# RaptorMai/online-continual-learning

Hardware: NVIDIA H100
Metric: replay-step images/sec (ASER+SCR, ResNet18, CIFAR100) (higher is better)
Workload: dtype f32

## Files before the change

### online-continual-learning_b200/csrc/umma.cuh

```cuda
#pragma once
#include <stdint.h>

namespace b200ocl {
namespace umma {

__device__ __forceinline__ uint32_t smem_u32(const void* p) {
  return static_cast<uint32_t>(__cvta_generic_to_shared(p));
}

__device__ __forceinline__ int sw128_offset_f32(int row, int chunk16) {
  return (row >> 3) * 256 + (row & 7) * 32 + ((chunk16 ^ (row & 7)) << 2);
}

__device__ __forceinline__ int frag_row(int t, int i) { return ((t >> 5) << 4) + ((t & 31) >> 2) + ((i & 2) << 2); }
__device__ __forceinline__ int frag_col(int t, int i) { return ((i >> 2) << 3) + ((t & 3) << 1) + (i & 1); }

__device__ __forceinline__ uint64_t make_smem_desc_sw128(uint32_t smem_addr) {
  uint64_t d = 0;
  d |= (uint64_t)((smem_addr >> 4) & 0x3FFF);
  d |= (uint64_t)1 << 16;
  d |= (uint64_t)((1024 >> 4) & 0x3FFF) << 32;
  d |= (uint64_t)1 << 62;
  return d;
}

__device__ __forceinline__ void fence() { asm volatile("wgmma.fence.sync.aligned;\n" ::: "memory"); }
__device__ __forceinline__ void commit() { asm volatile("wgmma.commit_group.sync.aligned;\n" ::: "memory"); }
template <int N>
__device__ __forceinline__ void wait() { asm volatile("wgmma.wait_group.sync.aligned %0;\n" ::"n"(N) : "memory"); }
template <int R>
__device__ __forceinline__ void fence_regs(float (&d)[R]) {
#pragma unroll
  for (int i = 0; i < R; ++i) asm volatile("" : "+f"(d[i])::"memory");
}
template <int N>
__device__ __forceinline__ void reg_dealloc() { asm volatile("setmaxnreg.dec.sync.aligned.u32 %0;\n" ::"n"(N)); }
template <int N>
__device__ __forceinline__ void reg_alloc() { asm volatile("setmaxnreg.inc.sync.aligned.u32 %0;\n" ::"n"(N)); }
__device__ __forceinline__ void fence_proxy_async_smem() { asm volatile("fence.proxy.async.shared::cta;\n" ::); }

__device__ __forceinline__ void mbar_init(uint64_t* bar, uint32_t count) {
  asm volatile("mbarrier.init.shared::cta.b64 [%0], %1;\n" ::"r"(smem_u32(bar)), "r"(count));
}
__device__ __forceinline__ void fence_mbar_init() { asm volatile("fence.mbarrier_init.release.cluster;\n" ::); }
__device__ __forceinline__ bool mbar_wait(uint64_t* bar, uint32_t parity, uint32_t max_spins = (1u << 24)) {
  const uint32_t addr = smem_u32(bar);
#pragma unroll 1
  for (uint32_t i = 0; i < max_spins; ++i) {
    uint32_t done;
    asm volatile(
        "{\n\t.reg .pred p;\n\t"
        "mbarrier.try_wait.parity.shared::cta.b64 p, [%1], %2;\n\t"
        "selp.u32 %0, 1, 0, p;\n\t}\n"
        : "=r"(done)
        : "r"(addr), "r"(parity)
        : "memory");
    if (done) return true;
  }
  return false;
}
__device__ __forceinline__ void mbar_arrive(uint64_t* bar) {
  asm volatile("mbarrier.arrive.shared::cta.b64 _, [%0];\n" ::"r"(smem_u32(bar)) : "memory");
}

__device__ __forceinline__ void mbar_expect_tx(uint64_t* bar, uint32_t bytes) {
  asm volatile("mbarrier.arrive.expect_tx.shared::cta.b64 _, [%0], %1;\n" ::"r"(smem_u32(bar)), "r"(bytes)
               : "memory");
}
__device__ __forceinline__ void bulk_g2s(void* smem_dst, const void* gmem_src, uint32_t bytes, uint64_t* bar) {
  asm volatile(
      "cp.async.bulk.shared::cluster.global.mbarrier::complete_tx::bytes [%0], [%1], %2, [%3];\n" ::"r"(
          smem_u32(smem_dst)),
      "l"(gmem_src), "r"(bytes), "r"(smem_u32(bar))
      : "memory");
}

__device__ __forceinline__ bool elect_one_sync() {
  uint32_t pred;
  asm volatile(
      "{\n\t.reg .pred P;\n\t"
      "elect.sync _|P, 0xffffffff;\n\t"
      "selp.u32 %0, 1, 0, P;\n\t}\n"
      : "=r"(pred));
  return pred != 0;
}

template <int N>
__device__ __forceinline__ void mma_tf32_ss(float (&d)[N / 2], uint64_t desc_a, uint64_t desc_b, uint32_t accumulate);
template <int N>
__device__ __forceinline__ void mma_tf32_rs(float (&d)[N / 2], const uint32_t (&a)[4], uint64_t desc_b, uint32_t accumulate);

template <>
__device__ __forceinline__ void mma_tf32_ss<16>(float (&d)[8], uint64_t desc_a, uint64_t desc_b, uint32_t accumulate) {
  asm volatile(
      "{\n\t.reg .pred p;\n\t"
      "setp.ne.b32 p, %10, 0;\n\t"
      "wgmma.mma_async.sync.aligned.m64n16k8.f32.tf32.tf32 {%0,%1,%2,%3,%4,%5,%6,%7}, %8, %9, p, 1, 1;\n\t}\n"
      : "+f"(d[0]), "+f"(d[1]), "+f"(d[2]), "+f"(d[3]), "+f"(d[4]), "+f"(d[5]), "+f"(d[6]), "+f"(d[7])
      : "l"(desc_a), "l"(desc_b), "r"(accumulate));
}

template <>
__device__ __forceinline__ void mma_tf32_ss<32>(float (&d)[16], uint64_t desc_a, uint64_t desc_b, uint32_t accumulate) {
  asm volatile(
      "{\n\t.reg .pred p;\n\t"
      "setp.ne.b32 p, %18, 0;\n\t"
      "wgmma.mma_async.sync.aligned.m64n32k8.f32.tf32.tf32 {%0,%1,%2,%3,%4,%5,%6,%7,%8,%9,%10,%11,%12,%13,%14,%15}, %16, %17, p, 1, 1;\n\t}\n"
      : "+f"(d[0]), "+f"(d[1]), "+f"(d[2]), "+f"(d[3]), "+f"(d[4]), "+f"(d[5]), "+f"(d[6]), "+f"(d[7]), "+f"(d[8]), "+f"(d[9]), "+f"(d[10]), "+f"(d[11]), "+f"(d[12]), "+f"(d[13]), "+f"(d[14]), "+f"(d[15])
      : "l"(desc_a), "l"(desc_b), "r"(accumulate));
}

template <>
__device__ __forceinline__ void mma_tf32_ss<48>(float (&d)[24], uint64_t desc_a, uint64_t desc_b, uint32_t accumulate) {
  asm volatile(
      "{\n\t.reg .pred p;\n\t"
      "setp.ne.b32 p, %26, 0;\n\t"
      "wgmma.mma_async.sync.aligned.m64n48k8.f32.tf32.tf32 {%0,%1,%2,%3,%4,%5,%6,%7,%8,%9,%10,%11,%12,%13,%14,%15,%16,%17,%18,%19,%20,%21,%22,%23}, %24, %25, p, 1, 1;\n\t}\n"
      : "+f"(d[0]), "+f"(d[1]), "+f"(d[2]), "+f"(d[3]), "+f"(d[4]), "+f"(d[5]), "+f"(d[6]), "+f"(d[7]), "+f"(d[8]), "+f"(d[9]), "+f"(d[10]), "+f"(d[11]), "+f"(d[12]), "+f"(d[13]), "+f"(d[14]), "+f"(d[15]), "+f"(d[16]), "+f"(d[17]), "+f"(d[18]), "+f"(d[19]), "+f"(d[20]), "+f"(d[21]), "+f"(d[22]), "+f"(d[23])
      : "l"(desc_a), "l"(desc_b), "r"(accumulate));
}

template <>
__device__ __forceinline__ void mma_tf32_ss<80>(float (&d)[40], uint64_t desc_a, uint64_t desc_b, uint32_t accumulate) {
  asm volatile(
      "{\n\t.reg .pred p;\n\t"
      "setp.ne.b32 p, %42, 0;\n\t"
      "wgmma.mma_async.sync.aligned.m64n80k8.f32.tf32.tf32 {%0,%1,%2,%3,%4,%5,%6,%7,%8,%9,%10,%11,%12,%13,%14,%15,%16,%17,%18,%19,%20,%21,%22,%23,%24,%25,%26,%27,%28,%29,%30,%31,%32,%33,%34,%35,%36,%37,%38,%39}, %40, %41, p, 1, 1;\n\t}\n"
      : "+f"(d[0]), "+f"(d[1]), "+f"(d[2]), "+f"(d[3]), "+f"(d[4]), "+f"(d[5]), "+f"(d[6]), "+f"(d[7]), "+f"(d[8]), "+f"(d[9]), "+f"(d[10]), "+f"(d[11]), "+f"(d[12]), "+f"(d[13]), "+f"(d[14]), "+f"(d[15]), "+f"(d[16]), "+f"(d[17]), "+f"(d[18]), "+f"(d[19]), "+f"(d[20]), "+f"(d[21]), "+f"(d[22]), "+f"(d[23]), "+f"(d[24]), "+f"(d[25]), "+f"(d[26]), "+f"(d[27]), "+f"(d[28]), "+f"(d[29]), "+f"(d[30]), "+f"(d[31]), "+f"(d[32]), "+f"(d[33]), "+f"(d[34]), "+f"(d[35]), "+f"(d[36]), "+f"(d[37]), "+f"(d[38]), "+f"(d[39])
      : "l"(desc_a), "l"(desc_b), "r"(accumulate));
}

template <>
__device__ __forceinline__ void mma_tf32_rs<32>(float (&d)[16], const uint32_t (&a)[4], uint64_t desc_b, uint32_t accumulate) {
  asm volatile(
      "{\n\t.reg .pred p;\n\t"
      "setp.ne.b32 p, %21, 0;\n\t"
      "wgmma.mma_async.sync.aligned.m64n32k8.f32.tf32.tf32 {%0,%1,%2,%3,%4,%5,%6,%7,%8,%9,%10,%11,%12,%13,%14,%15}, {%16,%17,%18,%19}, %20, p, 1, 1;\n\t}\n"
      : "+f"(d[0]), "+f"(d[1]), "+f"(d[2]), "+f"(d[3]), "+f"(d[4]), "+f"(d[5]), "+f"(d[6]), "+f"(d[7]), "+f"(d[8]), "+f"(d[9]), "+f"(d[10]), "+f"(d[11]), "+f"(d[12]), "+f"(d[13]), "+f"(d[14]), "+f"(d[15])
      : "r"(a[0]), "r"(a[1]), "r"(a[2]), "r"(a[3]), "l"(desc_b), "r"(accumulate));
}

__device__ __forceinline__ float round_tf32(float x) {
  uint32_t r;
  asm("cvt.rna.tf32.f32 %0, %1;\n" : "=r"(r) : "f"(x));
  return __uint_as_float(r);
}
__device__ __forceinline__ void split_tf32(float x, float& hi, float& lo) {
  hi = round_tf32(x);
  lo = x - hi;
}

}
}
```

### online-continual-learning_b200/csrc/wgrad_tc.cu

```cuda
#include "common.cuh"
#include "umma.cuh"
#include "wgrad_tc.cuh"

namespace b200ocl {
namespace {

constexpr int WT_THREADS = 32 * 14;
constexpr int WT_PS = 2;
constexpr int WT_XP = 40;
constexpr int WT_DZ_BYTES = 128 * 128;

struct WtGeom {
  int wp, pp, prow, xbytes;
};
__host__ __device__ inline WtGeom wt_geom(int H, int W) {
  WtGeom g;
  g.wp = W + 2;
  g.pp = (H + 2) * (W + 2);
  g.prow = 128 + 2 * g.wp + 2;
  g.xbytes = ((g.prow + 1) * WT_XP * 4 + 1023) / 1024 * 1024;
  return g;
}

__device__ __forceinline__ void load_a(const float* xs, int r, int c, uint32_t (&hi)[4], uint32_t (&lo)[4]) {
  const float v[4] = {xs[r * WT_XP + c], xs[r * WT_XP + c + 8], xs[(r + 4) * WT_XP + c], xs[(r + 4) * WT_XP + c + 8]};
#pragma unroll
  for (int i = 0; i < 4; ++i) {
    float h, l;
    umma::split_tf32(v[i], h, l);
    hi[i] = __float_as_uint(h);
    lo[i] = __float_as_uint(l);
  }
}

__global__ void __launch_bounds__(WT_THREADS, 1) wgrad_tc_kernel(WgradTcArgs a, int tiles_m) {
  extern __shared__ __align__(1024) unsigned char smem_raw[];
  __shared__ __align__(8) uint64_t full[WT_PS], empty[WT_PS];
  __shared__ int s_fail;

  const int tid = threadIdx.x, warp = tid >> 5, lane = tid & 31;
  const WtGeom G = wt_geom(a.H, a.W);
  const int stage_bytes = 2 * WT_DZ_BYTES + G.xbytes;
  const int sl = blockIdx.y, cb = blockIdx.z;
  const int chain0 = blockIdx.x * a.chains_per_cta;
  const int chain1 = min(a.chains, chain0 + a.chains_per_cta);
  const int k_total = 9 * a.Cin;

  if (tid == 0) {
    for (int i = 0; i < WT_PS; ++i) {
      umma::mbar_init(&full[i], 128 + 64);
      umma::mbar_init(&empty[i], 8);
    }
    umma::fence_mbar_init();
    s_fail = 0;
  }
  __syncthreads();

  if (warp >= 12) {
    const int lt = tid - 32 * 12;
    const int ch = lt & 7, r0 = lt >> 3;
    const bool ch_real = cb * 32 + ch * 4 < a.Cout;
    const int hp = a.H + 2;
    int pc = 0;
    for (int chain = chain0; chain < chain1; ++chain) {
      const int t1 = min(tiles_m, (chain + 1) * a.tpc);
      for (int tile = chain * a.tpc; tile < t1; ++tile, ++pc) {
        float4 v[16];
        int img, yp, xp;
        {
          const int sp = tile * 128 + r0;
          img = sp / G.pp;
          const int rem = sp - img * G.pp;
          yp = rem / G.wp;
          xp = rem - yp * G.wp;
        }
#pragma unroll
        for (int i = 0; i < 16; ++i) {
          v[i] = make_float4(0.f, 0.f, 0.f, 0.f);
          if (ch_real && img < a.N && yp < a.H && xp < a.W)
            v[i] = __ldg(reinterpret_cast<const float4*>(a.dz + ((size_t)(img * a.H + yp) * a.W + xp) * a.Cout + cb * 32) + ch);
          xp += 8;
          while (xp >= G.wp) {
            xp -= G.wp;
            if (++yp == hp) {
              yp = 0;
              ++img;
            }
          }
        }
        const int ps = pc % WT_PS;
        if (!umma::mbar_wait(&empty[ps], (uint32_t)(((pc / WT_PS) & 1) ^ 1))) s_fail = 1;
        float* zh = reinterpret_cast<float*>(smem_raw + (size_t)ps * stage_bytes);
        float* zl = zh + WT_DZ_BYTES / 4;
#pragma unroll
        for (int i = 0; i < 16; ++i) {
          const int pos = r0 + 8 * i;
          const float e[4] = {v[i].x, v[i].y, v[i].z, v[i].w};
#pragma unroll
          for (int j = 0; j < 4; ++j) {
            float h, l;
            umma::split_tf32(e[j], h, l);
            const int off = (pos >> 5) * 1024 + umma::sw128_offset_f32(ch * 4 + j, (pos & 31) >> 2) + (pos & 3);
            zh[off] = h;
            zl[off] = l;
          }
        }
        umma::fence_proxy_async_smem();
        umma::mbar_arrive(&full[ps]);
      }
    }
  } else if (warp >= 8) {
    const int lt = tid - 32 * 8;
    const int ch = lt & 7, r0 = lt >> 3;
    const int ch_valid = min(32, a.Cin - sl * 32);
    const bool ch_real = ch * 4 < ch_valid;
    const int nrow = G.prow;
    const int hp = a.H + 2;
    int pc = 0;
    for (int chain = chain0; chain < chain1; ++chain) {
      const int t1 = min(tiles_m, (chain + 1) * a.tpc);
      for (int tile = chain * a.tpc; tile < t1; ++tile, ++pc) {
        float4 v[WT_LD_MAX];
        int img, yp, xp;
        {
          const int sp = tile * 128 + r0;
          img = sp / G.pp;
          const int rem = sp - img * G.pp;
          yp = rem / G.wp;
          xp = rem - yp * G.wp;
        }
#pragma unroll
        for (int i = 0; i < WT_LD_MAX; ++i) {
          v[i] = make_float4(0.f, 0.f, 0.f, 0.f);
          const int ri = r0 + 16 * i;
          if (ch_real && ri < nrow) {
            const int y = yp - 1, x = xp - 1;
            if (img < a.N && (unsigned)y < (unsigned)a.H && (unsigned)x < (unsigned)a.W)
              v[i] = __ldg(reinterpret_cast<const float4*>(a.x + ((size_t)(img * a.H + y) * a.W + x) * a.Cin + sl * 32) + ch);
          }
          xp += 16;
          while (xp >= G.wp) {
            xp -= G.wp;
            if (++yp == hp) {
              yp = 0;
              ++img;
            }
          }
        }
        const int ps = pc % WT_PS;
        if (!umma::mbar_wait(&empty[ps], (uint32_t)(((pc / WT_PS) & 1) ^ 1))) s_fail = 1;
        float* xs = reinterpret_cast<float*>(smem_raw + (size_t)ps * stage_bytes + 2 * WT_DZ_BYTES);
#pragma unroll
        for (int i = 0; i < WT_LD_MAX; ++i) {
          const int ri = r0 + 16 * i;
          if (ri < nrow) *reinterpret_cast<float4*>(xs + ri * WT_XP + ch * 4) = v[i];
        }
        umma::mbar_arrive(&full[ps]);
      }
    }
  } else {
    const int h = warp >> 2, wt = tid & 127;
    const int m0 = 64 * h + 16 * (warp & 3) + (lane >> 2);
    const int kw = m0 >> 5, c = m0 & 31, q = lane & 3;
    const int n_valid = min(32, a.Cout - cb * 32);
    int pc = 0;
    for (int chain = chain0; chain < chain1; ++chain) {
      float acc[3][16];
      const int t0 = chain * a.tpc, t1 = min(tiles_m, (chain + 1) * a.tpc);
      for (int tile = t0; tile < t1; ++tile, ++pc) {
        const int ps = pc % WT_PS;
        if (!umma::mbar_wait(&full[ps], (uint32_t)((pc / WT_PS) & 1))) s_fail = 1;
        const unsigned char* st = smem_raw + (size_t)ps * stage_bytes;
        const float* xs = reinterpret_cast<const float*>(st + 2 * WT_DZ_BYTES);
        const uint64_t dZ0 = umma::make_smem_desc_sw128(umma::smem_u32(st));
        constexpr uint32_t Z_LO = (uint32_t)WT_DZ_BYTES >> 4;
#pragma unroll 1
        for (int ks = 0; ks < 16; ++ks) {
          const uint64_t dZh = dZ0 + (uint64_t)((ks >> 2) * 256 + (ks & 3) * 2), dZl = dZh + Z_LO;
          uint32_t ah[3][4], al[3][4];
#pragma unroll
          for (int kh = 0; kh < 3; ++kh) load_a(xs, ks * 8 + q + kh * G.wp + kw, c, ah[kh], al[kh]);
          const uint32_t accumulate = (tile == t0 && ks == 0) ? 0u : 1u;
          umma::fence();
#pragma unroll
          for (int kh = 0; kh < 3; ++kh) {
            umma::mma_tf32_rs<32>(acc[kh], ah[kh], dZh, accumulate);
            umma::mma_tf32_rs<32>(acc[kh], ah[kh], dZl, 1u);
            umma::mma_tf32_rs<32>(acc[kh], al[kh], dZh, 1u);
          }
          umma::commit();
          umma::wait<0>();
        }
#pragma unroll
        for (int kh = 0; kh < 3; ++kh) umma::fence_regs(acc[kh]);
        if (lane == 0) umma::mbar_arrive(&empty[ps]);
      }
#pragma unroll
      for (int i = 0; i < 16; i += 2) {
        const int m = 64 * h + umma::frag_row(wt, i), co = umma::frag_col(wt, i);
        const int kwi = m >> 5, ci = sl * 32 + (m & 31);
        if (kwi < 3 && ci < a.Cin && co < n_valid) {
#pragma unroll
          for (int kh = 0; kh < 3; ++kh) {
            float* dst = a.part + ((size_t)chain * k_total + (size_t)(kh * 3 + kwi) * a.Cin + ci) * a.Cout + cb * 32 + co;
            *reinterpret_cast<float2*>(dst) = make_float2(acc[kh][i], acc[kh][i + 1]);
          }
        }
      }
    }
  }
  __syncthreads();
  if (s_fail && tid == 0) a.part[0] = __int_as_float(0x7fc00000);
}

__global__ void wgrad_tc_reduce_kernel(const float* __restrict__ part, int chains, int Cin, int Cout, float* __restrict__ dw) {
  const int e = blockIdx.x * blockDim.x + threadIdx.x;
  const int total = 9 * Cin * Cout;
  if (e >= total) return;
  const int k = e / Cout, co = e - k * Cout;
  const int tap = k / Cin, ci = k - tap * Cin;
  double s = 0.0;
  for (int sp = 0; sp < chains; ++sp) s += (double)part[(size_t)sp * total + e];
  dw[((size_t)co * Cin + ci) * 9 + tap] = (float)s;
}

}

int launch_wgrad_tc(const WgradTcArgs& a, const WgradTcCfg& g, cudaStream_t stream) {
  const WtGeom G = wt_geom(a.H, a.W);
  const size_t smem = (size_t)WT_PS * (2 * WT_DZ_BYTES + (size_t)G.xbytes) + 1024;
  B200OCL_CUDA(raise_smem_limit<wgrad_tc_kernel>(smem));
  const double M = (double)a.N * a.H * a.W;
  B200OCL_PROF("wgrad_tc", 2.0 * M * 9.0 * a.Cin * a.Cout, stream);
  wgrad_tc_kernel<<<dim3(g.ctas_x, g.slices, g.cout_blocks), WT_THREADS, smem, stream>>>(a, g.tiles);
  B200OCL_LAUNCHED();
  return B200OCL_OK;
}

}

extern "C" size_t b200ocl_wgrad_tc_selftest_workspace_bytes(int N, int H, int W, int cin, int cout) {
  using namespace b200ocl;
  if (N < 1 || H < 1 || W < 1 || cin < 1 || cout < 1) return 0;
  const WgradTcCfg g = wgrad_tc_cfg(N, H, W, 3, 1, 1, cin, cout, sm_count());
  if (!g.eligible) return 0;
  return align_up((size_t)g.chains * 9 * cin * cout * sizeof(float), 256);
}

extern "C" int b200ocl_wgrad_tc_selftest(const float* x, const float* dz, float* dw_oihw, int N, int H, int W, int cin, int cout,
                                         void* workspace, size_t workspace_bytes, void* stream_) {
  using namespace b200ocl;
  cudaStream_t stream = static_cast<cudaStream_t>(stream_);
  B200OCL_CHECK_ARG(x && dz && dw_oihw && N >= 1, "null pointer / empty batch");
  const WgradTcCfg g = wgrad_tc_cfg(N, H, W, 3, 1, 1, cin, cout, sm_count());
  if (!g.eligible) {
    set_error("b200ocl_wgrad_tc_selftest: geometry not covered (3x3 stride 1, W <= 37, channels %% 4 == 0)");
    return B200OCL_EUNSUPPORTED;
  }
  int rc = check_workspace("b200ocl_wgrad_tc_selftest", workspace, workspace_bytes,
                           b200ocl_wgrad_tc_selftest_workspace_bytes(N, H, W, cin, cout));
  if (rc) return rc;
  WgradTcArgs a{};
  a.x = x; a.dz = dz; a.part = static_cast<float*>(workspace);
  a.N = N; a.H = H; a.W = W; a.Cin = cin; a.Cout = cout;
  a.tpc = g.tpc; a.chains = g.chains; a.chains_per_cta = g.chains_per_cta;
  if ((rc = launch_wgrad_tc(a, g, stream))) return rc;
  const int total = 9 * cin * cout;
  wgrad_tc_reduce_kernel<<<(total + 255) / 256, 256, 0, stream>>>(a.part, g.chains, cin, cout, dw_oihw);
  B200OCL_LAUNCHED();
  return B200OCL_OK;
}
```

### online-continual-learning_b200/csrc/wgrad_tc.cuh

```cuda
#pragma once
#include <cuda_runtime.h>

namespace b200ocl {

constexpr int WT_LD_MAX = 13;

struct WgradTcCfg {
  int eligible;
  int slices;
  int cout_blocks;
  int tiles;
  int tpc;
  int chains;
  int chains_per_cta;
  int ctas_x;
};

inline int wgrad_tc_tiles(int N, int H, int W) {
  const long pp = (long)(H + 2) * (W + 2);
  const long last = (long)(N - 1) * pp + (long)(H - 1) * (W + 2) + (W - 1);
  return (int)(last / 128) + 1;
}

inline WgradTcCfg wgrad_tc_cfg(int N, int H, int W, int ks, int stride, int pad, int cin, int cout, int sms) {
  WgradTcCfg g{};
  g.eligible = (ks == 3 && stride == 1 && pad == 1 && cin % 4 == 0 && cout % 4 == 0 && cin >= 4 && cout >= 4 &&
                128 + 2 * (W + 2) + 2 <= 16 * WT_LD_MAX && (long)N * (H + 2) * (W + 2) < 2000000000L) ? 1 : 0;
  if (!g.eligible) return g;
  g.slices = (cin + 31) / 32;
  g.cout_blocks = (cout + 31) / 32;
  g.tiles = wgrad_tc_tiles(N, H, W);
  g.tpc = 2;
  g.chains = (g.tiles + g.tpc - 1) / g.tpc;
  int want = sms / (g.slices * g.cout_blocks);
  if (want < 1) want = 1;
  if (want > g.chains) want = g.chains;
  g.chains_per_cta = (g.chains + want - 1) / want;
  g.ctas_x = (g.chains + g.chains_per_cta - 1) / g.chains_per_cta;
  return g;
}

struct WgradTcArgs {
  const float* x;
  const float* dz;
  float* part;
  int N, H, W, Cin, Cout;
  int tpc, chains, chains_per_cta;
};

int launch_wgrad_tc(const WgradTcArgs& a, const WgradTcCfg& g, cudaStream_t stream);

}
```

Measured before the change: 2186.

## Restructure wgrad tensor-core kernel with variable N tiles and two consumer groups

Reworks the 3x3 weight-gradient wgmma kernel. The input-channel slice drops from 32 to 20 so all three kw taps fit in one 64-row M tile, and the output-channel tile becomes a templated 8-40 multiple chosen to fit Cout with less padding. The two consumer warpgroups now process independent chains, each with its own staged buffers (up to four stages), instead of splitting M. A/B fragment loads are double-buffered against in-flight wgmma groups (wait<1>), and register allocation is rebalanced with setmaxnreg. This adds template instantiations and more complex stage indexing, and it changes the grid shape (more slices), which could shift load balance.

Result: faster. 2343 (median of 6 runs) (+7.1%).

```diff
diff --git a/online-continual-learning_b200/csrc/umma.cuh b/online-continual-learning_b200/csrc/umma.cuh
--- a/online-continual-learning_b200/csrc/umma.cuh
+++ b/online-continual-learning_b200/csrc/umma.cuh
@@ -140,6 +140,46 @@
       : "r"(a[0]), "r"(a[1]), "r"(a[2]), "r"(a[3]), "l"(desc_b), "r"(accumulate));
 }
 
+template <>
+__device__ __forceinline__ void mma_tf32_rs<8>(float (&d)[4], const uint32_t (&a)[4], uint64_t desc_b, uint32_t accumulate) {
+  asm volatile(
+      "{\n\t.reg .pred p;\n\t"
+      "setp.ne.b32 p, %9, 0;\n\t"
+      "wgmma.mma_async.sync.aligned.m64n8k8.f32.tf32.tf32 {%0,%1,%2,%3}, {%4,%5,%6,%7}, %8, p, 1, 1;\n\t}\n"
+      : "+f"(d[0]), "+f"(d[1]), "+f"(d[2]), "+f"(d[3])
+      : "r"(a[0]), "r"(a[1]), "r"(a[2]), "r"(a[3]), "l"(desc_b), "r"(accumulate));
+}
+
+template <>
+__device__ __forceinline__ void mma_tf32_rs<16>(float (&d)[8], const uint32_t (&a)[4], uint64_t desc_b, uint32_t accumulate) {
+  asm volatile(
+      "{\n\t.reg .pred p;\n\t"
+      "setp.ne.b32 p, %13, 0;\n\t"
+      "wgmma.mma_async.sync.aligned.m64n16k8.f32.tf32.tf32 {%0,%1,%2,%3,%4,%5,%6,%7}, {%8,%9,%10,%11}, %12, p, 1, 1;\n\t}\n"
+      : "+f"(d[0]), "+f"(d[1]), "+f"(d[2]), "+f"(d[3]), "+f"(d[4]), "+f"(d[5]), "+f"(d[6]), "+f"(d[7])
+      : "r"(a[0]), "r"(a[1]), "r"(a[2]), "r"(a[3]), "l"(desc_b), "r"(accumulate));
+}
+
+template <>
+__device__ __forceinline__ void mma_tf32_rs<24>(float (&d)[12], const uint32_t (&a)[4], uint64_t desc_b, uint32_t accumulate) {
+  asm volatile(
+      "{\n\t.reg .pred p;\n\t"
+      "setp.ne.b32 p, %17, 0;\n\t"
+      "wgmma.mma_async.sync.aligned.m64n24k8.f32.tf32.tf32 {%0,%1,%2,%3,%4,%5,%6,%7,%8,%9,%10,%11}, {%12,%13,%14,%15}, %16, p, 1, 1;\n\t}\n"
+      : "+f"(d[0]), "+f"(d[1]), "+f"(d[2]), "+f"(d[3]), "+f"(d[4]), "+f"(d[5]), "+f"(d[6]), "+f"(d[7]), "+f"(d[8]), "+f"(d[9]), "+f"(d[10]), "+f"(d[11])
+      : "r"(a[0]), "r"(a[1]), "r"(a[2]), "r"(a[3]), "l"(desc_b), "r"(accumulate));
+}
+
+template <>
+__device__ __forceinline__ void mma_tf32_rs<40>(float (&d)[20], const uint32_t (&a)[4], uint64_t desc_b, uint32_t accumulate) {
+  asm volatile(
+      "{\n\t.reg .pred p;\n\t"
+      "setp.ne.b32 p, %25, 0;\n\t"
+      "wgmma.mma_async.sync.aligned.m64n40k8.f32.tf32.tf32 {%0,%1,%2,%3,%4,%5,%6,%7,%8,%9,%10,%11,%12,%13,%14,%15,%16,%17,%18,%19}, {%20,%21,%22,%23}, %24, p, 1, 1;\n\t}\n"
+      : "+f"(d[0]), "+f"(d[1]), "+f"(d[2]), "+f"(d[3]), "+f"(d[4]), "+f"(d[5]), "+f"(d[6]), "+f"(d[7]), "+f"(d[8]), "+f"(d[9]), "+f"(d[10]), "+f"(d[11]), "+f"(d[12]), "+f"(d[13]), "+f"(d[14]), "+f"(d[15]), "+f"(d[16]), "+f"(d[17]), "+f"(d[18]), "+f"(d[19])
+      : "r"(a[0]), "r"(a[1]), "r"(a[2]), "r"(a[3]), "l"(desc_b), "r"(accumulate));
+}
+
 __device__ __forceinline__ float round_tf32(float x) {
   uint32_t r;
   asm("cvt.rna.tf32.f32 %0, %1;\n" : "=r"(r) : "f"(x));
diff --git a/online-continual-learning_b200/csrc/wgrad_tc.cu b/online-continual-learning_b200/csrc/wgrad_tc.cu
--- a/online-continual-learning_b200/csrc/wgrad_tc.cu
+++ b/online-continual-learning_b200/csrc/wgrad_tc.cu
@@ -5,10 +5,12 @@
 namespace b200ocl {
 namespace {
 
-constexpr int WT_THREADS = 32 * 14;
-constexpr int WT_PS = 2;
-constexpr int WT_XP = 40;
-constexpr int WT_DZ_BYTES = 128 * 128;
+constexpr int WT_THREADS = 32 * 16;
+constexpr int WT_PS_MAX = 4;
+constexpr int WT_XP = 24;
+constexpr size_t WT_SMEM_LIMIT = 227 * 1024 - 1024;
+
+__host__ __device__ constexpr int wt_dz_bytes(int bn) { return 4 * bn * 128; }
 
 struct WtGeom {
   int wp, pp, prow, xbytes;
@@ -18,191 +20,206 @@
   g.wp = W + 2;
   g.pp = (H + 2) * (W + 2);
   g.prow = 128 + 2 * g.wp + 2;
-  g.xbytes = ((g.prow + 1) * WT_XP * 4 + 1023) / 1024 * 1024;
+  g.xbytes = (g.prow * WT_XP * 4 + 1023) / 1024 * 1024;
   return g;
 }
 
-__device__ __forceinline__ void load_a(const float* xs, int r, int c, uint32_t (&hi)[4], uint32_t (&lo)[4]) {
-  const float v[4] = {xs[r * WT_XP + c], xs[r * WT_XP + c + 8], xs[(r + 4) * WT_XP + c], xs[(r + 4) * WT_XP + c + 8]};
-#pragma unroll
-  for (int i = 0; i < 4; ++i) {
-    float h, l;
-    umma::split_tf32(v[i], h, l);
-    hi[i] = __float_as_uint(h);
-    lo[i] = __float_as_uint(l);
-  }
-}
-
-__global__ void __launch_bounds__(WT_THREADS, 1) wgrad_tc_kernel(WgradTcArgs a, int tiles_m) {
+__host__ __device__ inline int wt_stage_bytes(const WtGeom& G, int bn) { return 2 * wt_dz_bytes(bn) + G.xbytes; }
+
+__device__ __forceinline__ void load_a(const float* xs, int p, int wp, int o0, int o1, uint32_t (&hi)[3][4],
+                                       uint32_t (&lo)[3][4]) {
+#pragma unroll
+  for (int kh = 0; kh < 3; ++kh) {
+    const float* r = xs + (p + kh * wp) * WT_XP;
+    const float v[4] = {r[o0], r[o1], r[4 * WT_XP + o0], r[4 * WT_XP + o1]};
+#pragma unroll
+    for (int i = 0; i < 4; ++i) {
+      float h, l;
+      umma::split_tf32(v[i], h, l);
+      hi[kh][i] = __float_as_uint(h);
+      lo[kh][i] = __float_as_uint(l);
+    }
+  }
+}
+
+template <int BN>
+__device__ __forceinline__ void issue_step(float (&acc)[3][BN / 2], const uint32_t (&hi)[3][4], const uint32_t (&lo)[3][4],
+                                           uint64_t dZh, uint64_t dZl, uint32_t accumulate) {
+  umma::fence();
+#pragma unroll
+  for (int kh = 0; kh < 3; ++kh) {
+    umma::mma_tf32_rs<BN>(acc[kh], hi[kh], dZh, accumulate);
+    umma::mma_tf32_rs<BN>(acc[kh], hi[kh], dZl, 1u);
+    umma::mma_tf32_rs<BN>(acc[kh], lo[kh], dZh, 1u);
+  }
+  umma::commit();
+}
+
+__device__ __forceinline__ int wt_row_kw(int m) { return min(m / WT_SLICE, 2); }
+
+template <int BN>
+__global__ void __launch_bounds__(WT_THREADS, 1) wgrad_tc_kernel(WgradTcArgs a, int tiles_m, int stages) {
   extern __shared__ __align__(1024) unsigned char smem_raw[];
-  __shared__ __align__(8) uint64_t full[WT_PS], empty[WT_PS];
+  __shared__ __align__(8) uint64_t full[WT_PS_MAX], empty[WT_PS_MAX];
   __shared__ int s_fail;
+  constexpr int DZ_BYTES = wt_dz_bytes(BN);
+  constexpr int SUB = BN * 128;
 
   const int tid = threadIdx.x, warp = tid >> 5, lane = tid & 31;
   const WtGeom G = wt_geom(a.H, a.W);
-  const int stage_bytes = 2 * WT_DZ_BYTES + G.xbytes;
+  const int stage_bytes = wt_stage_bytes(G, BN);
+  const int per = stages >> 1;
   const int sl = blockIdx.y, cb = blockIdx.z;
   const int chain0 = blockIdx.x * a.chains_per_cta;
   const int chain1 = min(a.chains, chain0 + a.chains_per_cta);
   const int k_total = 9 * a.Cin;
 
   if (tid == 0) {
-    for (int i = 0; i < WT_PS; ++i) {
-      umma::mbar_init(&full[i], 128 + 64);
-      umma::mbar_init(&empty[i], 8);
+    for (int i = 0; i < stages; ++i) {
+      umma::mbar_init(&full[i], 128 + 128);
+      umma::mbar_init(&empty[i], 4);
     }
     umma::fence_mbar_init();
     s_fail = 0;
   }
   __syncthreads();
 
-  if (warp >= 12) {
-    const int lt = tid - 32 * 12;
-    const int ch = lt & 7, r0 = lt >> 3;
-    const bool ch_real = cb * 32 + ch * 4 < a.Cout;
-    const int hp = a.H + 2;
-    int pc = 0;
-    for (int chain = chain0; chain < chain1; ++chain) {
-      const int t1 = min(tiles_m, (chain + 1) * a.tpc);
-      for (int tile = chain * a.tpc; tile < t1; ++tile, ++pc) {
-        float4 v[16];
-        int img, yp, xp;
-        {
-          const int sp = tile * 128 + r0;
-          img = sp / G.pp;
-          const int rem = sp - img * G.pp;
-          yp = rem / G.wp;
-          xp = rem - yp * G.wp;
+  if (warp >= 8) {
+    umma::reg_dealloc<96>();
+    const bool dz_loader = warp >= 12;
+    int pc0 = 0, pc1 = 0;
+    for (int c2 = chain0; c2 < chain1; c2 += 2) {
+      for (int tt = 0; tt < a.tpc; ++tt) {
+#pragma unroll 1
+        for (int h = 0; h < 2; ++h) {
+          const int chain = c2 + h, tile = chain * a.tpc + tt;
+          if (chain >= chain1 || tile >= tiles_m) continue;
+          const int n = h ? pc1++ : pc0++;
+          const int ps = h + 2 * (n % per);
+          const uint32_t parity = (uint32_t)(((n / per) & 1) ^ 1);
+          unsigned char* st = smem_raw + (size_t)ps * stage_bytes;
+          if (dz_loader) {
+            const int pos = tid - 32 * 12;
+            constexpr int NC = BN / 4;
+            float4 v[NC];
+            {
+              const int sp = tile * 128 + pos;
+              const int img = sp / G.pp, rem = sp - img * G.pp;
+              const int yp = rem / G.wp, xp = rem - yp * G.wp;
+              const bool pix = img < a.N && yp < a.H && xp < a.W;
+              const float* src = a.dz + ((size_t)(img * a.H + yp) * a.W + xp) * a.Cout + cb * BN;
+#pragma unroll
+              for (int j = 0; j < NC; ++j) {
+                v[j] = make_float4(0.f, 0.f, 0.f, 0.f);
+                if (pix && cb * BN + 4 * j < a.Cout) v[j] = __ldg(reinterpret_cast<const float4*>(src) + j);
+              }
+            }
+            if (!umma::mbar_wait(&empty[ps], parity)) s_fail = 1;
+            float* zh = reinterpret_cast<float*>(st);
+            float* zl = zh + DZ_BYTES / 4;
+#pragma unroll
+            for (int j = 0; j < NC; ++j) {
+              const float e[4] = {v[j].x, v[j].y, v[j].z, v[j].w};
+#pragma unroll
+              for (int k = 0; k < 4; ++k) {
+                float hv, lv;
+                umma::split_tf32(e[k], hv, lv);
+                const int off = (pos >> 5) * (SUB / 4) + umma::sw128_offset_f32(4 * j + k, (pos & 31) >> 2) + (pos & 3);
+                zh[off] = hv;
+                zl[off] = lv;
+              }
+            }
+            umma::fence_proxy_async_smem();
+          } else {
+            const int lt = tid - 32 * 8;
+            const int ch = lt & 7, r0 = lt >> 3;
+            const bool ch_real = ch * 4 < min(WT_SLICE, a.Cin - sl * WT_SLICE);
+            const int hp = a.H + 2;
+            float4 v[WT_LD_MAX];
+            int img, yp, xp;
+            {
+              const int sp = tile * 128 + r0;
+              img = sp / G.pp;
+              const int rem = sp - img * G.pp;
+              yp = rem / G.wp;
+              xp = rem - yp * G.wp;
+            }
+#pragma unroll
+            for (int i = 0; i < WT_LD_MAX; ++i) {
+              v[i] = make_float4(0.f, 0.f, 0.f, 0.f);
+              const int ri = r0 + 16 * i;
+              if (ch_real && ri < G.prow) {
+                const int y = yp - 1, x = xp - 1;
+                if (img < a.N && (unsigned)y < (unsigned)a.H && (unsigned)x < (unsigned)a.W)
+                  v[i] = __ldg(reinterpret_cast<const float4*>(a.x + ((size_t)(img * a.H + y) * a.W + x) * a.Cin +
+                                                               sl * WT_SLICE + ch * 4));
+              }
+              xp += 16;
+              while (xp >= G.wp) {
+                xp -= G.wp;
+                if (++yp == hp) {
+                  yp = 0;
+                  ++img;
+                }
+              }
+            }
+            if (!umma::mbar_wait(&empty[ps], parity)) s_fail = 1;
+            float* xs = reinterpret_cast<float*>(st + 2 * DZ_BYTES);
+            if (ch < WT_XP / 4) {
+#pragma unroll
+              for (int i = 0; i < WT_LD_MAX; ++i) {
+                const int ri = r0 + 16 * i;
+                if (ri < G.prow) *reinterpret_cast<float4*>(xs + ri * WT_XP + ch * 4) = v[i];
+              }
+            }
+          }
+          umma::mbar_arrive(&full[ps]);
         }
-#pragma unroll
-        for (int i = 0; i < 16; ++i) {
-          v[i] = make_float4(0.f, 0.f, 0.f, 0.f);
-          if (ch_real && img < a.N && yp < a.H && xp < a.W)
-            v[i] = __ldg(reinterpret_cast<const float4*>(a.dz + ((size_t)(img * a.H + yp) * a.W + xp) * a.Cout + cb * 32) + ch);
-          xp += 8;
-          while (xp >= G.wp) {
-            xp -= G.wp;
-            if (++yp == hp) {
-              yp = 0;
-              ++img;
-            }
-          }
-        }
-        const int ps = pc % WT_PS;
-        if (!umma::mbar_wait(&empty[ps], (uint32_t)(((pc / WT_PS) & 1) ^ 1))) s_fail = 1;
-        float* zh = reinterpret_cast<float*>(smem_raw + (size_t)ps * stage_bytes);
-        float* zl = zh + WT_DZ_BYTES / 4;
-#pragma unroll
-        for (int i = 0; i < 16; ++i) {
-          const int pos = r0 + 8 * i;
-          const float e[4] = {v[i].x, v[i].y, v[i].z, v[i].w};
-#pragma unroll
-          for (int j = 0; j < 4; ++j) {
-            float h, l;
-            umma::split_tf32(e[j], h, l);
-            const int off = (pos >> 5) * 1024 + umma::sw128_offset_f32(ch * 4 + j, (pos & 31) >> 2) + (pos & 3);
-            zh[off] = h;
-            zl[off] = l;
-          }
-        }
-        umma::fence_proxy_async_smem();
-        umma::mbar_arrive(&full[ps]);
-      }
-    }
-  } else if (warp >= 8) {
-    const int lt = tid - 32 * 8;
-    const int ch = lt & 7, r0 = lt >> 3;
-    const int ch_valid = min(32, a.Cin - sl * 32);
-    const bool ch_real = ch * 4 < ch_valid;
-    const int nrow = G.prow;
-    const int hp = a.H + 2;
-    int pc = 0;
-    for (int chain = chain0; chain < chain1; ++chain) {
-      const int t1 = min(tiles_m, (chain + 1) * a.tpc);
-      for (int tile = chain * a.tpc; tile < t1; ++tile, ++pc) {
-        float4 v[WT_LD_MAX];
-        int img, yp, xp;
-        {
-          const int sp = tile * 128 + r0;
-          img = sp / G.pp;
-          const int rem = sp - img * G.pp;
-          yp = rem / G.wp;
-          xp = rem - yp * G.wp;
-        }
-#pragma unroll
-        for (int i = 0; i < WT_LD_MAX; ++i) {
-          v[i] = make_float4(0.f, 0.f, 0.f, 0.f);
-          const int ri = r0 + 16 * i;
-          if (ch_real && ri < nrow) {
-            const int y = yp - 1, x = xp - 1;
-            if (img < a.N && (unsigned)y < (unsigned)a.H && (unsigned)x < (unsigned)a.W)
-              v[i] = __ldg(reinterpret_cast<const float4*>(a.x + ((size_t)(img * a.H + y) * a.W + x) * a.Cin + sl * 32) + ch);
-          }
-          xp += 16;
-          while (xp >= G.wp) {
-            xp -= G.wp;
-            if (++yp == hp) {
-              yp = 0;
-              ++img;
-            }
-          }
-        }
-        const int ps = pc % WT_PS;
-        if (!umma::mbar_wait(&empty[ps], (uint32_t)(((pc / WT_PS) & 1) ^ 1))) s_fail = 1;
-        float* xs = reinterpret_cast<float*>(smem_raw + (size_t)ps * stage_bytes + 2 * WT_DZ_BYTES);
-#pragma unroll
-        for (int i = 0; i < WT_LD_MAX; ++i) {
-          const int ri = r0 + 16 * i;
-          if (ri < nrow) *reinterpret_cast<float4*>(xs + ri * WT_XP + ch * 4) = v[i];
-        }
-        umma::mbar_arrive(&full[ps]);
       }
     }
   } else {
+    umma::reg_alloc<160>();
     const int h = warp >> 2, wt = tid & 127;
-    const int m0 = 64 * h + 16 * (warp & 3) + (lane >> 2);
-    const int kw = m0 >> 5, c = m0 & 31, q = lane & 3;
-    const int n_valid = min(32, a.Cout - cb * 32);
+    const int g = 16 * (warp & 3) + (lane >> 2), q = lane & 3;
+    const int kw0 = wt_row_kw(g), kw1 = wt_row_kw(g + 8);
+    const int o0 = kw0 * WT_XP + g - WT_SLICE * kw0, o1 = kw1 * WT_XP + g + 8 - WT_SLICE * kw1;
+    const int n_valid = min(BN, a.Cout - cb * BN);
+    constexpr uint32_t Z_LO = (uint32_t)DZ_BYTES >> 4;
     int pc = 0;
-    for (int chain = chain0; chain < chain1; ++chain) {
-      float acc[3][16];
+    for (int chain = chain0 + h; chain < chain1; chain += 2) {
+      float acc[3][BN / 2];
       const int t0 = chain * a.tpc, t1 = min(tiles_m, (chain + 1) * a.tpc);
       for (int tile = t0; tile < t1; ++tile, ++pc) {
-        const int ps = pc % WT_PS;
-        if (!umma::mbar_wait(&full[ps], (uint32_t)((pc / WT_PS) & 1))) s_fail = 1;
+        const int ps = h + 2 * (pc % per);
+        if (!umma::mbar_wait(&full[ps], (uint32_t)((pc / per) & 1))) s_fail = 1;
         const unsigned char* st = smem_raw + (size_t)ps * stage_bytes;
-        const float* xs = reinterpret_cast<const float*>(st + 2 * WT_DZ_BYTES);
+        const float* xs = reinterpret_cast<const float*>(st + 2 * DZ_BYTES);
         const uint64_t dZ0 = umma::make_smem_desc_sw128(umma::smem_u32(st));
-        constexpr uint32_t Z_LO = (uint32_t)WT_DZ_BYTES >> 4;
+        auto dz_desc = [&](int ks) { return dZ0 + (uint64_t)(((ks >> 2) * SUB + (ks & 3) * 32) >> 4); };
+        uint32_t ah[2][3][4], al[2][3][4];
+        load_a(xs, q, G.wp, o0, o1, ah[0], al[0]);
 #pragma unroll 1
-        for (int ks = 0; ks < 16; ++ks) {
-          const uint64_t dZh = dZ0 + (uint64_t)((ks >> 2) * 256 + (ks & 3) * 2), dZl = dZh + Z_LO;
-          uint32_t ah[3][4], al[3][4];
-#pragma unroll
-          for (int kh = 0; kh < 3; ++kh) load_a(xs, ks * 8 + q + kh * G.wp + kw, c, ah[kh], al[kh]);
-          const uint32_t accumulate = (tile == t0 && ks == 0) ? 0u : 1u;
-          umma::fence();
-#pragma unroll
-          for (int kh = 0; kh < 3; ++kh) {
-            umma::mma_tf32_rs<32>(acc[kh], ah[kh], dZh, accumulate);
-            umma::mma_tf32_rs<32>(acc[kh], ah[kh], dZl, 1u);
-            umma::mma_tf32_rs<32>(acc[kh], al[kh], dZh, 1u);
-          }
-          umma::commit();
-          umma::wait<0>();
+        for (int ks = 0; ks < 16; ks += 2) {
+          issue_step<BN>(acc, ah[0], al[0], dz_desc(ks), dz_desc(ks) + Z_LO, (tile == t0 && ks == 0) ? 0u : 1u);
+          umma::wait<1>();
+          load_a(xs, (ks + 1) * 8 + q, G.wp, o0, o1, ah[1], al[1]);
+          issue_step<BN>(acc, ah[1], al[1], dz_desc(ks + 1), dz_desc(ks + 1) + Z_LO, 1u);
+          umma::wait<1>();
+          load_a(xs, min(ks + 2, 15) * 8 + q, G.wp, o0, o1, ah[0], al[0]);
         }
+        umma::wait<0>();
 #pragma unroll
         for (int kh = 0; kh < 3; ++kh) umma::fence_regs(acc[kh]);
         if (lane == 0) umma::mbar_arrive(&empty[ps]);
       }
 #pragma unroll
-      for (int i = 0; i < 16; i += 2) {
-        const int m = 64 * h + umma::frag_row(wt, i), co = umma::frag_col(wt, i);
-        const int kwi = m >> 5, ci = sl * 32 + (m & 31);
-        if (kwi < 3 && ci < a.Cin && co < n_valid) {
+      for (int i = 0; i < BN / 2; i += 2) {
+        const int m = umma::frag_row(wt, i), co = umma::frag_col(wt, i);
+        const int kwi = wt_row_kw(m), c = m - WT_SLICE * kwi, ci = sl * WT_SLICE + c;
+        if (c < WT_SLICE && ci < a.Cin && co < n_valid) {
 #pragma unroll
           for (int kh = 0; kh < 3; ++kh) {
-            float* dst = a.part + ((size_t)chain * k_total + (size_t)(kh * 3 + kwi) * a.Cin + ci) * a.Cout + cb * 32 + co;
+            float* dst = a.part + ((size_t)chain * k_total + (size_t)(kh * 3 + kwi) * a.Cin + ci) * a.Cout + cb * BN + co;
             *reinterpret_cast<float2*>(dst) = make_float2(acc[kh][i], acc[kh][i + 1]);
           }
         }
@@ -224,17 +241,32 @@
   dw[((size_t)co * Cin + ci) * 9 + tap] = (float)s;
 }
 
-}
-
-int launch_wgrad_tc(const WgradTcArgs& a, const WgradTcCfg& g, cudaStream_t stream) {
+template <int BN>
+int launch_bn(const WgradTcArgs& a, const WgradTcCfg& g, cudaStream_t stream) {
   const WtGeom G = wt_geom(a.H, a.W);
-  const size_t smem = (size_t)WT_PS * (2 * WT_DZ_BYTES + (size_t)G.xbytes) + 1024;
-  B200OCL_CUDA(raise_smem_limit<wgrad_tc_kernel>(smem));
+  const size_t stage = (size_t)wt_stage_bytes(G, BN);
+  const int stages = 4 * stage + 1024 <= WT_SMEM_LIMIT ? 4 : 2;
+  const size_t smem = stages * stage + 1024;
+  B200OCL_CUDA(raise_smem_limit<wgrad_tc_kernel<BN>>(smem));
   const double M = (double)a.N * a.H * a.W;
   B200OCL_PROF("wgrad_tc", 2.0 * M * 9.0 * a.Cin * a.Cout, stream);
-  wgrad_tc_kernel<<<dim3(g.ctas_x, g.slices, g.cout_blocks), WT_THREADS, smem, stream>>>(a, g.tiles);
+  wgrad_tc_kernel<BN><<<dim3(g.ctas_x, g.slices, g.cout_blocks), WT_THREADS, smem, stream>>>(a, g.tiles, stages);
   B200OCL_LAUNCHED();
   return B200OCL_OK;
+}
+
+}
+
+int launch_wgrad_tc(const WgradTcArgs& a, const WgradTcCfg& g, cudaStream_t stream) {
+  switch (g.bn) {
+    case 8: return launch_bn<8>(a, g, stream);
+    case 16: return launch_bn<16>(a, g, stream);
+    case 24: return launch_bn<24>(a, g, stream);
+    case 32: return launch_bn<32>(a, g, stream);
+    case 40: return launch_bn<40>(a, g, stream);
+  }
+  set_error("launch_wgrad_tc: no kernel for a %d-channel output block", g.bn);
+  return B200OCL_EUNSUPPORTED;
 }
 
 }
diff --git a/online-continual-learning_b200/csrc/wgrad_tc.cuh b/online-continual-learning_b200/csrc/wgrad_tc.cuh
--- a/online-continual-learning_b200/csrc/wgrad_tc.cuh
+++ b/online-continual-learning_b200/csrc/wgrad_tc.cuh
@@ -4,11 +4,14 @@
 namespace b200ocl {
 
 constexpr int WT_LD_MAX = 13;
+constexpr int WT_SLICE = 20;
+constexpr int WT_BN_MAX = 40;
 
 struct WgradTcCfg {
   int eligible;
   int slices;
   int cout_blocks;
+  int bn;
   int tiles;
   int tpc;
   int chains;
@@ -27,8 +30,9 @@
   g.eligible = (ks == 3 && stride == 1 && pad == 1 && cin % 4 == 0 && cout % 4 == 0 && cin >= 4 && cout >= 4 &&
                 128 + 2 * (W + 2) + 2 <= 16 * WT_LD_MAX && (long)N * (H + 2) * (W + 2) < 2000000000L) ? 1 : 0;
   if (!g.eligible) return g;
-  g.slices = (cin + 31) / 32;
-  g.cout_blocks = (cout + 31) / 32;
+  g.slices = (cin + WT_SLICE - 1) / WT_SLICE;
+  g.cout_blocks = (cout + WT_BN_MAX - 1) / WT_BN_MAX;
+  g.bn = ((cout + g.cout_blocks - 1) / g.cout_blocks + 7) / 8 * 8;
   g.tiles = wgrad_tc_tiles(N, H, W);
   g.tpc = 2;
   g.chains = (g.tiles + g.tpc - 1) / g.tpc;
@@ -36,6 +40,7 @@
   if (want < 1) want = 1;
   if (want > g.chains) want = g.chains;
   g.chains_per_cta = (g.chains + want - 1) / want;
+  if (g.chains_per_cta > 1) g.chains_per_cta += g.chains_per_cta & 1;
   g.ctas_x = (g.chains + g.chains_per_cta - 1) / g.chains_per_cta;
   return g;
 }
```
